# bark-simulator/planner-miqp

Hardware: AMD Instinct MI355X
Metric: MIQP solves/sec to 1% gap, 2-agent x 20-step x 32-region (higher is better)
Workload: dtype f64

## Files before the change

### planner_miqp_amd/csrc/as_onchip.hip

```cpp
namespace miqp {

#ifdef MIQP_PROFILE
#define ASP_T(var) const long long var = clock64()
#define ASP_ACC(k, t0, t1) asp_[k] += (unsigned long long)((t1) - (t0))
#else
#define ASP_T(var)
#define ASP_ACC(k, t0, t1)
#endif
constexpr int AS_MAXSTEP = 220;
constexpr double AS_VTOL = 1.0e-8;
constexpr double AS_DEP = 1.0e-8;
constexpr int AS_MT = 64;
constexpr int AS_MSTR = AS_MT * (AS_MT + 1) / 2;

__host__ __device__ constexpr bool as_shape_ok(int C, int N) { return (C == 1 || C == 2) && N >= 1 && N <= 2 * OC_NSL; }

template <int C> __device__ inline int as_col(int pq) { return C == 2 ? ((pq & 3) << 2) | (pq >> 2) : ((pq & 1) << 2) | (pq >> 1); }
template <int C> __device__ inline int as_pcol(int q) { return C == 2 ? ((q & 3) << 2) | (q >> 2) : ((q & 3) << 1) | (q >> 2); }

template <int C, int NSL, int GCAP = miqp::OC_GCAP>
__global__ void __launch_bounds__(64, (GCAP > 128 ? 1 : 2)) as_onchip_kernel(DevBuf B) {
  static_assert(C == 1 || C == 2, "a stage of 16 columns holds the chains of up to two cars");
  constexpr bool CM = true;
  constexpr bool BIG = GCAP > 128;
  constexpr int OC_GCAP = GCAP, OC_GSLOTS = OC_GCAP / 64, OC_GCOEF = oc_gcoef_of(OC_GCAP);
  constexpr int NX = 6 * C, NZ = 8 * C, NCH = 2 * C;
  const Layout& Y = B.Y;
  const int tid = threadIdx.x, lg = tid >> 4, lc = tid & 15;
  const int par = lg >> 1, side = lg & 1;
  const double bsgn = side ? -1.0 : 1.0;
  WAVE_DUMP(BIG ? 1 : 4);
  const int* const clist = BIG && B.cls_take ? B.cls_list + (size_t)(B.cls_take - 1) * B.batch_cap : nullptr;
  const int nbatch = clist ? (B.cls_count[B.cls_take - 1] < B.batch_cap ? B.cls_count[B.cls_take - 1] : B.batch_cap) : (*B.batch_count < B.batch_cap ? *B.batch_count : B.batch_cap);
  const int N = Y.N, NSLOT = Y.NSLOT;
  extern __shared__ double lds[];
  char* const L0 = (char*)lds;
  const OcLds LL = oc_lds_layout(N, Y.fixlen, OC_GCAP, !BIG);
  double* const Z = (double*)(L0 + LL.z);
  double* const scr = (double*)(L0 + LL.u);
  double* const V = (double*)(L0 + LL.u);
  unsigned long long* const bkey = (unsigned long long*)(L0 + LL.r);
  const int SPAN = LL.gmeta - LL.u;
  double* const kref = (double*)(L0 + LL.u + SPAN - N * 32);
  double* const kff = kref - N * 4;
  double* const KS = kff - N * 16;
  const int STG_CAP = (SPAN - N * 192) / 8;
  uint4* const gmeta = (uint4*)(L0 + LL.gmeta);
  double* const gcoef = (double*)(L0 + LL.gcoef);
  double* const grhs = (double*)(L0 + LL.grhs);
  double* const Wd = (double*)(L0 + LL.wd);
  int* const sstart = (int*)(L0 + LL.sstart);
  unsigned short* const cand = (unsigned short*)(L0 + LL.cand);
  signed char* const fix = (signed char*)(L0 + LL.fix);
  __shared__ int sh_node;
  __shared__ unsigned long long sh_stat[32];
  if (tid < 32) sh_stat[tid] = 0ull;
  const unsigned long long lt = (1ull << tid) - 1ull;

  const int chunk = B.as_chunk > 0 ? B.as_chunk : 1;
  int run_next = 0, run_end = 0;
  const int quota = BIG ? 0 : B.as_quota; int handed = 0;
#ifdef MIQP_PROFILE
  const unsigned long long wv_c0 = __builtin_amdgcn_s_memtime(), wv_r0 = __builtin_amdgcn_s_memrealtime();
  unsigned long long wv_first = 0; int wv_nodes = 0;
  if (!BIG && tid == 0) wv_first = atomicMin(&B.prof[120], wv_r0);
#endif
  for (;;) {
    __syncthreads();
    if (run_next >= run_end) {
      if (quota > 0 && handed >= quota) break;
      ++handed;
      if (tid == 0) sh_node = atomicAdd(B.work_counter, chunk);
      __syncthreads();
      run_next = __builtin_amdgcn_readfirstlane(sh_node); run_end = run_next + chunk;
      if (run_next >= nbatch) break;
    }
    const int slot_ = run_next++;
    if (slot_ >= nbatch) { run_next = run_end; continue; }
    const int node = clist ? __builtin_amdgcn_readfirstlane(clist[slot_]) : slot_;
    {
      const int cls = B.batch_large ? (int)B.batch_large[node] : (is_probe_word(B.batch_depth[node]) ? 1 : 0);
      if (cls != (BIG ? 1 : 0)) continue;
    }
    WAVE_DUMP_NODE();
    const int inst = __builtin_amdgcn_readfirstlane(B.batch_inst[node]);
    const double* D = B.inst_d + (size_t)inst * Y.dstride;
    const int* T = B.inst_i + (size_t)inst * Y.istride;
    const double ts = D[Y.d_glob + 7];
    const double aqs = 2.0 * D[Y.d_misc + 0];
    const double iaq = aqs > 0.0 ? 1.0 / aqs : 0.0;
    {
      const signed char* src = B.pool_fix + (size_t)B.batch_node[node] * Y.fixlen;
      for (int k = tid; k < Y.fixlen; k += 64) fix[k] = src[k];
      if (tid < 16) Wd[tid] = tid < NZ ? D[Y.d_wd + oc_lcol<C, CM>(as_pcol<C>(tid))] : 0.0;
      for (int k = tid; k < N * 32; k += 64) bkey[k] = ~0ull;
      for (int k = tid; k <= N + 1; k += 64) sstart[k] = 0;
    }
    __syncthreads();
    const double* Rf = D + Y.d_ref;
    double cutoff = 1e300;
    {
      const double inc0 = fmin(inc_from_key(*(volatile unsigned long long*)&B.inc_key[inst]), B.inc_ext[inst]);
      const double gap_ = is_probe_word(B.batch_depth[node]) ? 0.0 : B.inst_gap[inst];
      if (B.use_cutoff && inc0 < 1e300) cutoff = inc0 - gap_ * (1e-10 + fabs(inc0)) - B.inst_const[inst];
    }

#ifdef MIQP_PROFILE
    unsigned long long asp_[12] = {0, 0, 0, 0, 0, 0, 0, 0, 0, 0, 0, 0};
#endif
    ASP_T(ta0);
    int ngen = 0;
    {
      unsigned long long* const bmp = (unsigned long long*)scr;
      const int nw = (N * NSLOT + 63) >> 6;
      unsigned short* const pre = (unsigned short*)(bmp + nw);
      for (int k = tid; k < nw; k += 64) bmp[k] = 0ull;
      OC_WAVE_SYNC();
      const int cls_off[8] = {0, 7, 11, 16, 16 + Y.EL, 16 + 5 * Y.EL, C * Y.SC, C * Y.SC + 8 * Y.NP};
      const int cls_cnt[8] = {7, 4, 5, Y.EL, 4 * Y.EL, 5 * Y.O, 8 * Y.NP, 16 * Y.NP};
      auto take = [&](int i, int slot) {
        if (decode_row<C, false>(Y, D, T, fix, i, slot, nullptr).active) {
          int col; double sg, rh;
          if (box_of_slot<C>(Y, D, T, fix, i, slot, col, sg, rh)) atomicMin(&bkey[(i * 2 + (sg < 0.0 ? 1 : 0)) * 16 + as_col<C>(oc_pcol<C, CM>(col))], d2key(rh));
          else { const int pcode = i * NSLOT + slot; atomicOr(&bmp[pcode >> 6], 1ull << (pcode & 63)); }
        }
      };
      unsigned short* const plist = pre + ((nw + 1 + 3) & ~3);
      const int LCAP = (int)(((char*)(L0 + LL.r) - (char*)plist) / 2) - 64;
      int nlist = 0;
      auto flush = [&]() {
        OC_WAVE_SYNC();
        for (int j0 = 0; j0 < nlist; j0 += 64) if (j0 + tid < nlist) { const int pc = plist[j0 + tid]; const int i = pc / NSLOT; take(i, pc - i * NSLOT); }
        OC_WAVE_SYNC();
        nlist = 0;
      };
      for (int e0 = 0; e0 < C * N; e0 += 64) {
        const int e = e0 + tid;
        if (e < C * N) {
          const int c = e / N, i = e - c * N;
          const double* G = D + Y.d_glob;
          const int code = i >= 1 ? (int)fix[Y.f_reg + c * N + i] : -1;
          const unsigned int skip = i >= 1 ? (unsigned int)T[Y.i_boxskip + c * N + i] : 0x7Fu;
          const double* rt = code >= 0 ? D + Y.d_reg + (c * Y.P + (code >> 2)) * REGSZ : nullptr;
          const double* Hc = (!rt && i >= 1) ? region_hull(Y, D, T, fix, c, i) : nullptr;
          auto put = [&](int col, bool neg, double rh) { atomicMin(&bkey[(i * 2 + (neg ? 1 : 0)) * 16 + as_col<C>(oc_pcol<C, CM>(col))], d2key(rh)); };
          if (i >= 1) {
            const double a_lo_x = rt ? rt[11] : Hc[0], a_hi_x = rt ? rt[12] : Hc[1], a_lo_y = rt ? rt[13] : Hc[2], a_hi_y = rt ? rt[14] : Hc[3];
            if (!(skip & 1u)) put(6 * c + 1, true, -G[0]);
            if (!(skip & 2u)) put(6 * c + 4, true, -G[0]);
            if (!(skip & 4u)) put(6 * c + 1, false, G[1]);
            if (!(skip & 8u)) put(6 * c + 2, false, a_hi_x);
            if (!(skip & 16u)) put(6 * c + 2, true, -a_lo_x);
            if (!(skip & 32u)) put(6 * c + 5, false, a_hi_y);
            if (!(skip & 64u)) put(6 * c + 5, true, -a_lo_y);
          }
          if (i <= N - 2) {
#pragma unroll
            for (int s_ = 0; s_ < 2; ++s_) {
              double lo, hi;
              if (i == 0) { lo = D[Y.d_u0box + c * 4 + 2 * s_]; hi = D[Y.d_u0box + c * 4 + 2 * s_ + 1]; }
              else if (rt) { lo = rt[15 + 2 * s_]; hi = rt[16 + 2 * s_]; }
              else { lo = Hc[4 + 2 * s_]; hi = Hc[5 + 2 * s_]; }
              put(6 * C + 2 * c + s_, false, hi); put(6 * C + 2 * c + s_, true, -lo);
            }
          }
        }
      }
#pragma unroll 1
      for (int cl = 0; cl < 8; ++cl) {
#ifdef MIQP_PROFILE
        if (cl == 2) { const long long tq_ = clock64(); asp_[9] += (unsigned long long)(tq_ - ta0); }
#endif
        const int cnt = cls_cnt[cl], off = cls_off[cl];
        const bool percar = cl < 6;
        const int per = percar ? C * cnt : cnt, total = N * per;
        for (int e0 = 0; e0 < total; e0 += 64) {
          const int e = e0 + tid;
          int i = 0, slot = 0; bool in = e < total;
          if (in) { i = e / per; const int rem = e - i * per; slot = percar ? (rem / cnt) * Y.SC + off + rem % cnt : off + rem; }
          if (cl < 2) continue;
          const bool cnd = in && slot_maybe<C>(Y, fix, i, slot);
          const unsigned long long mk = __ballot(cnd);
          if (cnd) plist[nlist + __popcll(mk & lt)] = (unsigned short)(i * NSLOT + slot);
          nlist += __popcll(mk);
          if (nlist > LCAP) flush();
        }
      }
      flush();
      if (tid == 0) { int a = 0; for (int k = 0; k < nw; ++k) { pre[k] = (unsigned short)(a < 65535 ? a : 65535); a += __popcll(bmp[k]); } pre[nw] = (unsigned short)(a < 65535 ? a : 65535); }
      OC_WAVE_SYNC();
      ngen = pre[nw];
      if (ngen <= OC_GCAP)
        for (int k = tid; k < nw; k += 64) {
          unsigned long long bits = bmp[k]; int pos = pre[k];
          while (bits) { const int b = __ffsll((long long)bits) - 1; cand[pos++] = (unsigned short)(k * 64 + b); bits &= bits - 1ull; }
        }
      OC_WAVE_SYNC();
    }
#ifdef MIQP_PROFILE
    const long long tq1_ = clock64();
#endif
    bool overflow = ngen > OC_GCAP;
    int ncoef = 0;
    for (int c0 = 0; c0 < ngen && !overflow; c0 += OC_SCR) {
      double* g = scr + (tid & (OC_SCR - 1)) * OC_SSTR;
      RowOut r; r.active = false; r.rhs = 0; r.aq = 0;
      int i = 0, nn = 0;
      const bool mine = tid < OC_SCR && c0 + tid < ngen;
      int slot_ = 0;
      if (mine) { const int pcode = cand[c0 + tid]; i = pcode / NSLOT; slot_ = pcode - i * NSLOT; r = decode_row<C, true>(Y, D, T, fix, i, slot_, g); }
      unsigned long long map = 0ull; unsigned int cols = 0u;
      double v6[6];
#pragma unroll
      for (int k = 0; k < 6; ++k) v6[k] = 0.0;
      if (mine) {
        for (int q = 0; q < NZ; ++q) {
          const double v = g[q];
          if (v != 0.0 && nn < 6) {
#pragma unroll
            for (int k = 0; k < 6; ++k) if (k == nn) v6[k] = v;
            const int pq = as_col<C>(oc_pcol<C, CM>(q));
            map |= (unsigned long long)(nn + 1) << (4 * pq); cols |= (unsigned int)pq << (4 * nn); nn++;
          }
        }
      }
      const bool keep = mine && nn > 0;
      const unsigned long long mk = __ballot(keep);
      const unsigned long long b0 = __ballot(keep && (nn & 1)), b1 = __ballot(keep && (nn & 2)), b2 = __ballot(keep && (nn & 4));
      const int tot = __popcll(b0) + 2 * __popcll(b1) + 4 * __popcll(b2);
      if (ncoef + tot > OC_GCOEF) { overflow = true; break; }
      if (keep) {
        const int idx = sstart[N + 1] + __popcll(mk & lt);
        const int off = ncoef + __popcll(b0 & lt) + 2 * __popcll(b1 & lt) + 4 * __popcll(b2 & lt);
#pragma unroll
        for (int k = 0; k < 6; ++k) if (k < nn) gcoef[off + k] = v6[k];
        uint4 m4; m4.x = (unsigned int)map; m4.y = (unsigned int)(map >> 32);
        m4.z = (unsigned int)off | ((unsigned int)nn << 16) | ((unsigned int)i << 20) | (r.aq > 0.0 ? 0x80000000u : 0u); m4.w = cols;
        gmeta[idx] = m4; grhs[idx] = r.rhs;
        cand[idx] = (unsigned short)(i * NSLOT + slot_);
      }
      OC_WAVE_SYNC();
      if (tid == 0) sstart[N + 1] += __popcll(mk);
      ncoef += tot;
      OC_WAVE_SYNC();
    }
    if (overflow) {
      if (B.batch_A) B.batch_A[(size_t)node * 64 + tid] = 0xFFFFu;
      if (tid == 0) {
        if (B.ring_M) B.batch_Mtag[node] = 0ull;
        B.batch_ok[node] = 5; B.pool_big[B.batch_node[node]] |= (BIG ? 2 : 1); if (B.stats) { atomicAdd(&B.stats[3], 1ull); atomicAdd(&B.stats[8 + (ngen >= 512 ? 15 : ngen / 32)], 1ull); }
      }
      continue;
    }
    const int NM = sstart[N + 1];
    OC_WAVE_SYNC();

    ASP_T(ta1); ASP_ACC(0, ta0, ta1);
#ifdef MIQP_PROFILE
    asp_[11] += (unsigned long long)(ta1 - tq1_);
#endif
    double brhs[NSL];
    unsigned int bact = 0u, binA = 0u, ginA = 0u;
#pragma unroll
    for (int k = 0; k < NSL; ++k) {
      const int i = 2 * k + par;
      brhs[k] = 1e300;
      if (i < N && lc < NZ) {
        const unsigned long long key = bkey[(i * 2 + side) * 16 + lc];
        if (key != ~0ull) { brhs[k] = key2d(key); bact |= 1u << k; }
      }
    }
    OC_WAVE_SYNC();

    const double h1 = ts, h2 = 0.5 * ts * ts, h3 = ts * ts * ts / 6.0;
    const double* const tb = D + Y.d_astab;
    if constexpr (C == 2) {
      for (int k = tid; k < N * 16; k += 64) KS[k] = tb[k];
      for (int k = tid; k < N * 4; k += 64) kref[k] = tb[N * 16 + k];
    } else {
      for (int k = tid; k < N * 8; k += 64) KS[(k >> 3) * 16 + (k & 7)] = tb[k];
      for (int k = tid; k < N * 2; k += 64) kref[(k >> 1) * 4 + (k & 1)] = tb[N * 8 + k];
    }
    OC_WAVE_SYNC();
    typedef double d2_t __attribute__((ext_vector_type(2)));
    auto subst = [&](const bool fromx0, const int itop, const int iend, double* const out) {
      for (int k = tid; k < (N - 1) * 4; k += 64) if ((k >> 2) > itop) kff[k] = fromx0 ? kref[k] : 0.0;
      if (tid < NCH) {
        const int ch = tid;
        double p0 = 0.0, p1 = 0.0, p2 = 0.0;
        int i0 = itop;
        if (itop >= N - 1) { const d2_t a = *(const d2_t*)(V + (N - 1) * 16 + 4 * ch); p0 = a[0]; p1 = a[1]; p2 = V[(N - 1) * 16 + 4 * ch + 2]; i0 = N - 2; }
        if (i0 >= 0) {
          d2_t va = *(const d2_t*)(V + i0 * 16 + 4 * ch), vb = *(const d2_t*)(V + i0 * 16 + 4 * ch + 2);
          d2_t ka = *(const d2_t*)(KS + (i0 * 4 + ch) * 4), kb = *(const d2_t*)(KS + (i0 * 4 + ch) * 4 + 2);
          double kr = fromx0 ? kref[i0 * 4 + ch] : 0.0;
          for (int i = i0; i >= 0; --i) {
            const int j = i > 0 ? i - 1 : 0;
            const d2_t nva = *(const d2_t*)(V + j * 16 + 4 * ch), nvb = *(const d2_t*)(V + j * 16 + 4 * ch + 2);
            const d2_t nka = *(const d2_t*)(KS + (j * 4 + ch) * 4), nkb = *(const d2_t*)(KS + (j * 4 + ch) * 4 + 2);
            const double nkr = fromx0 ? kref[j * 4 + ch] : 0.0;
            const double su = vb[1] + h3 * p0 + h2 * p1 + h1 * p2;
            const double sx0 = va[0] + p0, sx1 = va[1] + h1 * p0 + p1, sx2 = vb[0] + h2 * p0 + h1 * p1 + p2;
            kff[i * 4 + ch] = fma(su, kb[1], kr);
            p0 = sx0 - ka[0] * su; p1 = sx1 - ka[1] * su; p2 = sx2 - kb[0] * su;
            va = nva; vb = nvb; ka = nka; kb = nkb; kr = nkr;
          }
        }
      }
      OC_WAVE_SYNC();
      if (tid < NCH) {
        const int ch = tid;
        double x0 = 0.0, x1 = 0.0, x2 = 0.0;
        if (fromx0) { const int c = ch >> 1, s = ch & 1; x0 = D[Y.d_x0 + 6 * c + 3 * s]; x1 = D[Y.d_x0 + 6 * c + 3 * s + 1]; x2 = D[Y.d_x0 + 6 * c + 3 * s + 2]; }
        const int ie = iend < N - 1 ? iend : N - 2;
        d2_t ka = *(const d2_t*)(KS + ch * 4), kb = *(const d2_t*)(KS + ch * 4 + 2);
        double kf = kff[ch];
        for (int i = 0; i <= ie; ++i) {
          const int j = i < N - 2 ? i + 1 : N - 2;
          const d2_t nka = *(const d2_t*)(KS + (j * 4 + ch) * 4), nkb = *(const d2_t*)(KS + (j * 4 + ch) * 4 + 2);
          const double nkf = kff[j * 4 + ch];
          const double u = -kf - (ka[0] * x0 + ka[1] * x1 + kb[0] * x2);
          d2_t oa, ob; oa[0] = x0; oa[1] = x1; ob[0] = x2; ob[1] = u;
          *(d2_t*)(out + i * 16 + 4 * ch) = oa; *(d2_t*)(out + i * 16 + 4 * ch + 2) = ob;
          const double n0 = x0 + h1 * x1 + h2 * x2 + h3 * u, n1 = x1 + h1 * x2 + h2 * u, n2 = x2 + h1 * u;
          x0 = n0; x1 = n1; x2 = n2;
          ka = nka; kb = nkb; kf = nkf;
        }
        if (iend >= N - 1 || ie == N - 2) { d2_t oa, ob; oa[0] = x0; oa[1] = x1; ob[0] = x2; ob[1] = 0.0; *(d2_t*)(out + (ie + 1) * 16 + 4 * ch) = oa; *(d2_t*)(out + (ie + 1) * 16 + 4 * ch + 2) = ob; }
// ... 434 lines not shown
```

### planner_miqp_amd/csrc/solve_diag.hpp

```cpp
#pragma once

inline void debug_sync(hipStream_t st, int round, const char* stage, int nodes = -1) {
  hipError_t e_ = hipStreamSynchronize(st);
  if (nodes >= 0) std::fprintf(stderr, "[dbg] round %d %s (%d nodes): %s\n", round, stage, nodes, hipGetErrorString(e_));
  else std::fprintf(stderr, "[dbg] round %d %s: %s\n", round, stage, hipGetErrorString(e_));
}

inline bool trace_selection(const DevCtx& X, int rounds, int bc) {
  const DevBuf& B = X.B;
  std::vector<double> sb(bc); std::vector<int> sd(bc); double io_ = 0; int md_ = 0;
  HIP_OK(hipMemcpy(sb.data(), B.batch_bound, (size_t)bc * 8, hipMemcpyDeviceToHost)); HIP_OK(hipMemcpy(sd.data(), B.batch_depth, (size_t)bc * 4, hipMemcpyDeviceToHost));
  HIP_OK(hipMemcpy(&io_, B.inc_obj, 8, hipMemcpyDeviceToHost)); HIP_OK(hipMemcpy(&md_, B.inst_mode, 4, hipMemcpyDeviceToHost));
  std::vector<int> ord(bc); for (int k = 0; k < bc; ++k) ord[k] = k;
  std::sort(ord.begin(), ord.end(), [&](int a, int b) { return sd[a] != sd[b] ? sd[a] > sd[b] : sb[a] < sb[b]; });
  std::fprintf(stderr, "[sel] r%d mode %d incumbent %a:", rounds, md_, io_);
  for (int k : ord) std::fprintf(stderr, " %d.%d/%a", sd[k] >> 6, sd[k] & 63, sb[k]);
  std::fprintf(stderr, "\n");
  return true;
}

inline bool trace_batch(const DevCtx& X, int rounds, int bc) {
  const DevBuf& B = X.B; hipStream_t st = X.stream;
  HIP_OK(hipStreamSynchronize(st));
  if (X.stream2) HIP_OK(hipStreamSynchronize(X.stream2));
// ... 36 lines not shown
  hipEvent_t e0, e1; HIP_OK(hipEventCreate(&e0)); HIP_OK(hipEventCreate(&e1));
  HIP_OK(hipEventRecord(e0, st));
  for (int r = 0; r < replay; ++r) launch_ipm_batch(X, B, bc, st);
  HIP_OK(hipEventRecord(e1, st)); HIP_OK(hipStreamSynchronize(st));
  float ms = 0; HIP_OK(hipEventElapsedTime(&ms, e0, e1));
  std::vector<int> its(bc); HIP_OK(hipMemcpy(its.data(), B.batch_it, (size_t)bc * 4, hipMemcpyDeviceToHost));
  long long tot = 0; for (int v : its) tot += v;
  std::fprintf(stderr, "[miqp_gpu replay] %d nodes, %lld node-iterations: %.3f ms per pass, %.1f ns per node-iteration\n", bc, tot, ms / replay, 1e6 * ms / replay / (double)tot);
#ifdef MIQP_ABLATE
  if (X.oc_grid > 0 && Y.C == 2) {
    const size_t l_oc = (size_t)oc_lds_layout(Y.N, Y.fixlen).total;
    auto run = [&](auto kern, int mask) {
      HIP_OK(hipFuncSetAttribute((const void*)kern, hipFuncAttributeMaxDynamicSharedMemorySize, (int)l_oc));
      auto once = [&] { (void)hipMemsetAsync(B.work_counter, 0, 4, st); (void)hipMemsetAsync(B.ovf_count, 0, 4, st); hipLaunchKernelGGL(kern, dim3(std::min(bc, X.oc_grid)), dim3(64), l_oc, st, B); };
      once(); HIP_OK(hipEventRecord(e0, st)); for (int r = 0; r < 3; ++r) once(); HIP_OK(hipEventRecord(e1, st)); HIP_OK(hipStreamSynchronize(st));
      float m2 = 0; HIP_OK(hipEventElapsedTime(&m2, e0, e1));
      std::fprintf(stderr, "[miqp_gpu ablate] mask %4d: %.3f ms per pass of %d nodes x 15 iterations = %.1f ns per node-iteration\n", mask, m2 / 3, bc, 1e6 * m2 / 3 / (bc * 15.0));
      return true;
    };
    run(ipm_onchip_kernel<2, OC_NSL, 1>, 1); run(ipm_onchip_kernel<2, OC_NSL, 3>, 3); run(ipm_onchip_kernel<2, OC_NSL, 5>, 5); run(ipm_onchip_kernel<2, OC_NSL, 9>, 9);
    run(ipm_onchip_kernel<2, OC_NSL, 17>, 17); run(ipm_onchip_kernel<2, OC_NSL, 33>, 33); run(ipm_onchip_kernel<2, OC_NSL, 65>, 65); run(ipm_onchip_kernel<2, OC_NSL, 129>, 129);
    run(ipm_onchip_kernel<2, OC_NSL, 257>, 257); run(ipm_onchip_kernel<2, OC_NSL, 513>, 513); run(ipm_onchip_kernel<2, OC_NSL, 1023>, 1023);
    run(ipm_onchip_kernel<2, OC_NSL, 1025>, 1025);
    launch_ipm_batch(X, B, bc, st);
  }
#endif
  replay = 0;
  return true;
}

inline bool print_progress(const DevCtx& X, double t, int rounds, long long launched_nodes, double const0) {
  const DevBuf& B = X.B; hipStream_t st = X.stream;
  double lb0 = 0, io0 = 0; int oc0 = 0; unsigned long long k0 = 0;
  HIP_OK(hipMemcpyAsync(&lb0, B.lower_bound, 8, hipMemcpyDeviceToHost, st)); HIP_OK(hipMemcpyAsync(&io0, B.inc_obj, 8, hipMemcpyDeviceToHost, st));
  HIP_OK(hipMemcpyAsync(&oc0, B.open_count, 4, hipMemcpyDeviceToHost, st)); HIP_OK(hipMemcpyAsync(&k0, B.inc_key, 8, hipMemcpyDeviceToHost, st));
  int fc0 = 0; HIP_OK(hipMemcpyAsync(&fc0, B.far_count, 4, hipMemcpyDeviceToHost, st));
  HIP_OK(hipStreamSynchronize(st));
  std::fprintf(stderr, "[miqp_gpu] t %.2f s round %d nodes %lld: instance 0 bound %.4f incumbent %.4f open %d + %d\n", t, rounds, launched_nodes, lb0, k0 >= 0xFFF0000000000000ull ? INFINITY : io0 + const0, oc0, fc0);
  return true;
}

inline bool dump_open_list(const DevCtx& X, const char* dp, int rounds, int NS, double const0) {
  const DevBuf& B = X.B; const Layout& Y = X.Y; const int open_cap = X.open_cap;
  int oc0 = 0; HIP_OK(hipMemcpy(&oc0, B.open_count, 4, hipMemcpyDeviceToHost)); oc0 = std::min(oc0, open_cap);
  const size_t src = ((size_t)(rounds & 1) * NS + 0) * open_cap;
  std::vector<double> hb(oc0); std::vector<int> hn(oc0), hd(oc0);
  if (oc0 > 0) { HIP_OK(hipMemcpy(hb.data(), B.open_bound + src, (size_t)oc0 * 8, hipMemcpyDeviceToHost)); HIP_OK(hipMemcpy(hn.data(), B.open_node + src, (size_t)oc0 * 4, hipMemcpyDeviceToHost));
    HIP_OK(hipMemcpy(hd.data(), B.open_depth + src, (size_t)oc0 * 4, hipMemcpyDeviceToHost)); }
  std::vector<int> ord(oc0); for (int k = 0; k < oc0; ++k) ord[k] = k;
  std::sort(ord.begin(), ord.end(), [&](int x, int y) { return hb[x] < hb[y]; });
  if (FILE* f = std::fopen(dp, "w")) {
    std::fprintf(f, "%d %d %d %d %d %d %d\n", oc0, Y.fixlen, Y.f_reg, Y.f_env, Y.f_obs, Y.f_c2c, Y.N);
    std::vector<signed char> rec(Y.fixlen);
    for (int q = 0; q < std::min(oc0, 400); ++q) {
      int k = ord[q]; HIP_OK(hipMemcpy(rec.data(), B.pool_fix + (size_t)hn[k] * Y.fixlen, Y.fixlen, hipMemcpyDeviceToHost));
      std::fprintf(f, "%.9g %d", hb[k] + const0, hd[k] >> 6); for (int x = 0; x < Y.fixlen; ++x) std::fprintf(f, " %d", (int)rec[x]); std::fprintf(f, "\n");
    }
    std::fclose(f);
  }
  return true;
}

#ifdef MIQP_PROFILE
inline bool print_profile(const DevCtx& X) {
  const DevBuf& B = X.B;
  { unsigned long long pf[64]; HIP_OK(hipMemcpy(pf, B.prof + 64, 64 * 8, hipMemcpyDeviceToHost));
    const char* nm[10] = {"decode", "rowpass", "bw.phi", "bw.TS+p", "bw.readlane+LDL", "bw.Ksolve", "bw.update", "forward", "step", "update"};
    double tot = 0; for (int q = 0; q < 10; ++q) tot += (double)pf[q];
    { unsigned long long po[16]; HIP_OK(hipMemcpy(po, B.prof, 16 * 8, hipMemcpyDeviceToHost));
      const char* no[9] = {"build", "bw.rows/assemble", "bw.mfma", "bw.TS", "bw.cholK", "bw.P", "forward", "step", "update"};
      double to = 0; for (int q = 0; q < 9; ++q) to += (double)po[q];
      if (po[10]) { std::fprintf(stderr, "[miqp_gpu profile] memory-backed kernel nodes %llu iters %llu cycles/node-iter %.0f :", po[10], po[9], to / std::max(1ull, po[9]));
        for (int q = 0; q < 9; ++q) std::fprintf(stderr, " %s %.1f%% (%.0f)", no[q], 100.0 * po[q] / to, (double)po[q] / std::max(1ull, po[9]));
        std::fprintf(stderr, "; inside bw.TS, the stage-Hessian chain: weights + staging %.0f, single-entry rows %.0f, MFMA loop %.0f, reductions + diagonal %.0f", (double)po[12] / std::max(1ull, po[9]), (double)po[13] / std::max(1ull, po[9]), (double)po[14] / std::max(1ull, po[9]), (double)po[15] / std::max(1ull, po[9]));
        std::fprintf(stderr, "\n"); } }
    std::fprintf(stderr, "[miqp_gpu profile] on-chip nodes %llu iters %llu cycles/node-iter %.0f :", pf[11], pf[10], tot / std::max(1ull, pf[10]));
    for (int q = 0; q < 10; ++q) std::fprintf(stderr, " %s %.1f%% (%.0f)", nm[q], 100.0 * pf[q] / tot, (double)pf[q] / std::max(1ull, pf[10]));
    std::fprintf(stderr, "\n");
    { unsigned long long pa[14]; HIP_OK(hipMemcpy(pa, B.prof + 80, 14 * 8, hipMemcpyDeviceToHost));
      const char* na[9] = {"decode", "gains + first iterate", "scan", "response of the row", "q", "directions + ratio test + M update", "iterate refresh", "results", "warm start"};
      double ta = 0; for (int q = 0; q < 9; ++q) ta += (double)pa[q];
      if (pa[10]) { std::fprintf(stderr, "[miqp_gpu profile] active-set kernel nodes %llu steps %llu cycles/node %.0f :", pa[10], pa[11], ta / (double)pa[10]);
        for (int q = 0; q < 9; ++q) std::fprintf(stderr, " %s %.1f%% (%.0f)", na[q], 100.0 * pa[q] / ta, (double)pa[q] / (double)pa[10]);
        std::fprintf(stderr, "; inside the decode: bound classes %.0f, general-row pass %.0f", (double)pa[12] / (double)pa[10], (double)pa[13] / (double)pa[10]);
        std::fprintf(stderr, "\n");
        unsigned long long pw[3], pl[6]; HIP_OK(hipMemcpy(pw, B.prof + 94, 3 * 8, hipMemcpyDeviceToHost)); HIP_OK(hipMemcpy(pl, B.prof + 120, 6 * 8, hipMemcpyDeviceToHost));
        if (pw[2] && pw[1] && pl[5]) std::fprintf(stderr, "[miqp_gpu profile] standard active-set launches: %llu wavefronts resident %.0f shader cycles = %.1f us each (shader clock %.0f MHz); per launch (%llu folded): span %.3f ms, from the first wavefront out of work to the last end %.3f ms, wavefronts %.0f, resident wavefront time / (span x wavefronts) %.3f\n",
          pw[2], (double)pw[0] / pw[2], (double)pw[1] / pw[2] / 100.0, 100.0 * (double)pw[0] / (double)pw[1], pl[5], (double)pl[3] / pl[5] / 1e5, (double)pl[4] / pl[5] / 1e5, (double)pw[2] / pl[5], ((double)pw[1]) / ((double)pl[3] * ((double)pw[2] / pl[5])));
        unsigned long long ph[16]; HIP_OK(hipMemcpy(ph, B.prof + 128, 16 * 8, hipMemcpyDeviceToHost));
        if (pw[2]) { std::fprintf(stderr, "[miqp_gpu profile] standard active-set wavefronts by their start after the launch's first (< 0.05 / 0.2 / 0.5 / 1 / 2 / 4 / 8 ms / later), %% :");
          for (int q = 0; q < 8; ++q) std::fprintf(stderr, " %.1f", 100.0 * ph[q] / pw[2]);
          std::fprintf(stderr, "; by the nodes they solved (0 / <= 4 / <= 16 / <= 32 / <= 64 / more), %% :");
          for (int q = 8; q < 14; ++q) std::fprintf(stderr, " %.1f", 100.0 * ph[q] / pw[2]);
          std::fprintf(stderr, "\n"); }
        if (const char* wd = X.sw.wave_dump) {
          std::vector<unsigned long long> w(4 * 4 * 4096); HIP_OK(hipMemcpy(w.data(), B.prof + 160, w.size() * 8, hipMemcpyDeviceToHost));
          if (FILE* f = std::fopen(wd, "w")) { for (int q = 0; q < 4 * 4096; ++q) if (w[4 * q]) std::fprintf(f, "%d %llu %llu %u %u %llu %d\n", q & 4095, w[4 * q], w[4 * q + 1], (unsigned)(w[4 * q + 2] >> 32), (unsigned)w[4 * q + 2], w[4 * q + 3], q >> 12); std::fclose(f); } } } }
    { unsigned long long pe[8]; HIP_OK(hipMemcpy(pe, B.prof + 100, 8 * 8, hipMemcpyDeviceToHost));
      const char* ne[6] = {"load", "regions", "leaf disjunctions", "branching", "lifting + reservation", "records"};
      double te = 0; for (int q = 0; q < 6; ++q) te += (double)pe[q];
      if (pe[6]) { std::fprintf(stderr, "[miqp_gpu profile] eval_kernel, %llu branched nodes, cycles/node %.0f :", pe[6], te / (double)pe[6]);
        for (int q = 0; q < 6; ++q) std::fprintf(stderr, " %s %.1f%% (%.0f)", ne[q], 100.0 * pe[q] / te, (double)pe[q] / (double)pe[6]);
        std::fprintf(stderr, "\n"); } }
    { unsigned long long ps[10]; HIP_OK(hipMemcpy(ps, B.prof + 110, 10 * 8, hipMemcpyDeviceToHost));
      const char* ns[8] = {"incumbent copy / kill", "setup", "pass 1 (prune, keys)", "far refill", "bound reduce + spill select", "focus + window + share", "radix select + ties", "pass 3 (emit, compact)"};
      double ts = 0; for (int q = 0; q < 8; ++q) ts += (double)ps[q];
      if (ps[8]) { std::fprintf(stderr, "[miqp_gpu profile] select_kernel, %llu workgroups that reached the end (thread 0's clock), mean list %.0f entries, cycles each %.0f :", ps[8], (double)ps[9] / (double)ps[8], ts / (double)ps[8]);
        for (int q = 0; q < 8; ++q) std::fprintf(stderr, " %s %.1f%% (%.0f)", ns[q], 100.0 * ps[q] / ts, (double)ps[q] / (double)ps[8]);
        std::fprintf(stderr, "\n"); } }
    HIP_OK(hipMemset(B.prof, 0, 160 * 8)); }
  return true;
}
#endif

inline bool print_stats(const DevCtx& X) {
  const DevBuf& B = X.B; const Layout& Y = X.Y;
  unsigned long long hs[256]; HIP_OK(hipMemcpy(hs, B.stats, sizeof(hs), hipMemcpyDeviceToHost)); HIP_OK(hipMemset(B.stats, 0, sizeof(hs)));
  const double nn_ = (double)std::max(1ull, hs[0]);
  std::fprintf(stderr, "[miqp_gpu stats] on-chip nodes %llu (general rows %.1f, coefficients %.1f, box keys %.1f, iterations %.1f per node), handed over %llu; general rows / 32 histogram:", hs[0], hs[1] / nn_, hs[4] / nn_, hs[2] / nn_, hs[5] / nn_, hs[3]);
  for (int q = 0; q < 16; ++q) std::fprintf(stderr, " %llu", hs[8 + q]);
  std::fprintf(stderr, "\n");
  std::fprintf(stderr, "[miqp_gpu stats] node outcomes: infeasible %llu (%.1f it), cut off %llu (%.1f it), not converged %llu (%.1f it), solved %llu (%.1f it) of which: bound >= incumbent %llu, within gap %llu, integer feasible %llu, branched %llu (%.2f children; by kind region/env/obstacle/car-car: %llu x %.1f, %llu x %.1f, %llu x %.1f, %llu x %.1f)\n",
               hs[32], hs[36] / (double)std::max(1ull, hs[32]), hs[33], hs[37] / (double)std::max(1ull, hs[33]), hs[34], hs[38] / (double)std::max(1ull, hs[34]), hs[35], hs[39] / (double)std::max(1ull, hs[35]),
               hs[40], hs[41], hs[42], hs[43], hs[44] / (double)std::max(1ull, hs[43]), hs[48], hs[52] / (double)std::max(1ull, hs[48]), hs[49], hs[53] / (double)std::max(1ull, hs[49]),
               hs[50], hs[54] / (double)std::max(1ull, hs[50]), hs[51], hs[55] / (double)std::max(1ull, hs[51]));
  std::fprintf(stderr, "[miqp_gpu stats] region sets: tightened at %llu (car, step) sites, %llu nodes closed because a step had no region left; children not created because of their lifted bound %llu (multi-row lift larger than the single-row one: %llu), car/car sets tightened at %llu groups\n", hs[58], hs[59], hs[56], hs[57], hs[61]);
  std::fprintf(stderr, "[miqp_gpu stats] region branchings flagged by: own rows %llu (worst class acc box %llu, jerk box %llu, sector %llu, half-plane %llu, curvature %llu, slow square %llu), environment front rows %llu, obstacle front rows %llu, car/car front rows %llu; by step:",
               hs[64], hs[70], hs[71], hs[72], hs[73], hs[74], hs[75], hs[65], hs[66], hs[67]);
  for (int q = 0; q < 32 && q < Y.N; ++q) std::fprintf(stderr, " %llu", hs[160 + q]);
  std::fprintf(stderr, "\n[miqp_gpu stats] node outcomes by origin (processed: infeasible / cut off / not converged / solved):");
  const char* on_[16] = {"root|reg-ref", "reg-adjacent", "reg-other", "reg-slow", "env-ref", "env-other", "-", "-", "obs-ref", "obs-other", "-", "-", "c2c-ref", "c2c-other", "-", "probe"};
  for (int q = 0; q < 16; ++q) if (hs[80 + q]) std::fprintf(stderr, " %s %llu: %llu / %llu / %llu / %llu;", on_[q], hs[80 + q], hs[96 + q], hs[112 + q], hs[128 + q], hs[144 + q]);
  std::fprintf(stderr, "\n[miqp_gpu stats] infeasible rounding probes re-rounded: %llu", hs[62]);
  std::fprintf(stderr, "\n[miqp_gpu stats] handed-over nodes with >= 480 general rows: %llu, mean %.0f, most %llu general rows", hs[7], (double)hs[6] / std::max(1ull, hs[7]), hs[5]);
  std::fprintf(stderr, "\n[miqp_gpu stats] rounding probes by iterations / 3 (0-2, 3-5, ..., 45+):");
  { const char* oc_n[4] = {"infeasible", "cut off", "not converged", "solved"};
    for (int o = 0; o < 4; ++o) { std::fprintf(stderr, " %s", oc_n[o]); for (int q = 0; q < 16; ++q) std::fprintf(stderr, " %llu", hs[192 + 16 * o + q]); std::fprintf(stderr, ";"); } }
  std::fprintf(stderr, "\n");
  return true;
}

inline void print_as_stats(const unsigned long long* h_as) {
  std::fprintf(stderr, "[miqp_gpu stats] active-set launch: %llu nodes (%.1f steps, %.1f drops, %.1f rows from the parent's active set, %.1f active rows at the end per node; %llu infeasible, %llu cut off; %llu started from the parent's M, %llu fell back to a cold start), %llu handed to the interior point (no free slot %llu, step cap %llu, curvature %llu, down-date pivot %llu, rows off their equalities %llu, other %llu); M rebuilt because: the parent left none %llu, the ring had come round %llu, another row count %llu; in the larger block %llu nodes (%.1f steps), of them leaves of the local search %llu (%.1f steps), rounding probes %llu; by their general rows (<= 64 / 96 / 128 / 192 / more) %llu / %llu / %llu / %llu / %llu\n",
               h_as[0], h_as[1] / (double)std::max(1ull, h_as[0]), h_as[3] / (double)std::max(1ull, h_as[0]), h_as[7] / (double)std::max(1ull, h_as[0]), h_as[6] / (double)std::max(1ull, h_as[0]), h_as[4], h_as[5], h_as[8], h_as[9], h_as[2], h_as[11], h_as[12], h_as[13], h_as[14], h_as[15], h_as[10], h_as[17], h_as[18], h_as[19], h_as[20], h_as[21] / (double)std::max(1ull, h_as[20]), h_as[22], h_as[23] / (double)std::max(1ull, h_as[22]), h_as[29], h_as[24], h_as[25], h_as[26], h_as[27], h_as[28]);
}
```

Before: 1085.

## Decode constraint rows per lane-site with count-scan-write instead of slot enumeration

Replaces the slot-by-slot decode of the active-set kernel with a per-site decode: each lane owns one (step, car) or (step, pair) site, emits box bounds to atomic keys and counts general rows, then a wave prefix scan assigns output offsets and a second pass writes the packed rows. This removes the bitmap, candidate list, per-slot ballots and the scratch-based coefficient extraction loop. It decodes each site twice and leaves lanes idle when there are fewer sites than lanes. Under a debug macro the old path stays available and both images are hashed and compared.

Result: no change. 1098, median of 3 (+1.2%).

```diff
diff --git a/planner_miqp_amd/csrc/as_onchip.hip b/planner_miqp_amd/csrc/as_onchip.hip
--- a/planner_miqp_amd/csrc/as_onchip.hip
+++ b/planner_miqp_amd/csrc/as_onchip.hip
@@ -1,3 +1,5 @@
+#include "site_decode.hpp"
+
 namespace miqp {
 
 #ifdef MIQP_PROFILE
@@ -110,6 +112,120 @@
 #endif
     ASP_T(ta0);
     int ngen = 0;
+    bool overflow = false;
+    struct SdCount {
+      unsigned long long* bkey; int ncand, nkeep, ncoef;
+      __device__ void box(int i, int col, double sgn, double rhs) { atomicMin(&bkey[(i * 2 + (sgn < 0.0 ? 1 : 0)) * 16 + as_col<C>(oc_pcol<C, true>(col))], d2key(rhs)); }
+      __device__ void gen(int, int, double, double, int, double a0, double a1, double a2, double a3, double a4, double a5, int bb, double b0, double b1, double b2, double b3, double b4, double b5) {
+        int nn = (a0 != 0.0) + (a1 != 0.0) + (a2 != 0.0) + (a3 != 0.0) + (a4 != 0.0) + (a5 != 0.0);
+        if (bb >= 0) nn += (b0 != 0.0) + (b1 != 0.0) + (b2 != 0.0) + (b3 != 0.0) + (b4 != 0.0) + (b5 != 0.0);
+        if (nn > 6) nn = 6;
+        ++ncand;
+        if (nn > 0) { ++nkeep; ncoef += nn; }
+      }
+    };
+    struct SdWrite {
+      uint4* gmeta; double* gcoef; double* grhs; unsigned short* cand; int NSLOT, idx, off;
+      __device__ void box(int, int, double, double) {}
+      __device__ void gen(int i, int slot, double rhs, double aq, int ba, double a0, double a1, double a2, double a3, double a4, double a5, int bb, double b0, double b1, double b2, double b3, double b4, double b5) {
+        int nn = 0; unsigned long long map = 0ull; unsigned int cols = 0u;
+        auto put = [&](const int q, const double v) {
+          if (v != 0.0 && nn < 6) {
+            if (off + nn < OC_GCOEF) gcoef[off + nn] = v;
+            const int pq = as_col<C>(oc_pcol<C, true>(q));
+            map |= (unsigned long long)(nn + 1) << (4 * pq); cols |= (unsigned int)pq << (4 * nn); nn++;
+          }
+        };
+        put(ba, a0); put(ba + 1, a1); put(ba + 2, a2); put(ba + 3, a3); put(ba + 4, a4); put(ba + 5, a5);
+        if (bb >= 0) { put(bb, b0); put(bb + 1, b1); put(bb + 2, b2); put(bb + 3, b3); put(bb + 4, b4); put(bb + 5, b5); }
+        if (nn > 0 && idx < OC_GCAP) {
+          uint4 m4; m4.x = (unsigned int)map; m4.y = (unsigned int)(map >> 32);
+          m4.z = (unsigned int)off | ((unsigned int)nn << 16) | ((unsigned int)i << 20) | (aq > 0.0 ? 0x80000000u : 0u); m4.w = cols;
+          gmeta[idx] = m4; grhs[idx] = rhs; cand[idx] = (unsigned short)(i * NSLOT + slot);
+          ++idx; off += nn;
+        }
+      }
+    };
+#ifdef MIQP_PROFILE
+    long long tq1_ = 0;
+#endif
+    auto decode_sites = [&]() {
+      constexpr int SPS = C == 2 ? 3 : 1;
+      const int ln = fresh_lane();
+      const int si = ln / SPS, sj = ln - si * SPS;
+      const bool car_site = si < N && sj < C, pair_site = C == 2 && si < N && sj == C;
+      SdCount S1; S1.bkey = bkey; S1.ncand = 0; S1.nkeep = 0; S1.ncoef = 0;
+      if (car_site) {
+        const int c = sj, i = si;
+        const double* G = D + Y.d_glob;
+        const int code = i >= 1 ? (int)fix[Y.f_reg + c * N + i] : -1;
+        const unsigned int skip = i >= 1 ? (unsigned int)T[Y.i_boxskip + c * N + i] : 0x7Fu;
+        const double* rt = code >= 0 ? D + Y.d_reg + (c * Y.P + (code >> 2)) * REGSZ : nullptr;
+        const double* Hc = (!rt && i >= 1) ? region_hull(Y, D, T, fix, c, i) : nullptr;
+        auto put = [&](int col, bool neg, double rh) { atomicMin(&bkey[(i * 2 + (neg ? 1 : 0)) * 16 + as_col<C>(oc_pcol<C, CM>(col))], d2key(rh)); };
+        if (i >= 1) {
+          const double a_lo_x = rt ? rt[11] : Hc[0], a_hi_x = rt ? rt[12] : Hc[1], a_lo_y = rt ? rt[13] : Hc[2], a_hi_y = rt ? rt[14] : Hc[3];
+          if (!(skip & 1u)) put(6 * c + 1, true, -G[0]);
+          if (!(skip & 2u)) put(6 * c + 4, true, -G[0]);
+          if (!(skip & 4u)) put(6 * c + 1, false, G[1]);
+          if (!(skip & 8u)) put(6 * c + 2, false, a_hi_x);
+          if (!(skip & 16u)) put(6 * c + 2, true, -a_lo_x);
+          if (!(skip & 32u)) put(6 * c + 5, false, a_hi_y);
+          if (!(skip & 64u)) put(6 * c + 5, true, -a_lo_y);
+        }
+        if (i <= N - 2) {
+#pragma unroll
+          for (int s_ = 0; s_ < 2; ++s_) {
+            double lo, hi;
+            if (i == 0) { lo = D[Y.d_u0box + c * 4 + 2 * s_]; hi = D[Y.d_u0box + c * 4 + 2 * s_ + 1]; }
+            else if (rt) { lo = rt[15 + 2 * s_]; hi = rt[16 + 2 * s_]; }
+            else { lo = Hc[4 + 2 * s_]; hi = Hc[5 + 2 * s_]; }
+            put(6 * C + 2 * c + s_, false, hi); put(6 * C + 2 * c + s_, true, -lo);
+          }
+        }
+        site_rows_car<C>(Y, D, T, fix, c, i, S1);
+      } else if (pair_site) site_rows_pair<C>(Y, D, T, fix, 0, si, S1);
+      int pk = S1.nkeep, pc = S1.ncoef, pn = S1.ncand;
+#pragma unroll
+      for (int d = 1; d < 64; d <<= 1) {
+        const int tk = __shfl_up(pk, d), tc = __shfl_up(pc, d), tn = __shfl_up(pn, d);
+        if (tid >= d) { pk += tk; pc += tc; pn += tn; }
+      }
+      ngen = __shfl(pn, 63);
+      const int nkeep = __shfl(pk, 63), ncoef = __shfl(pc, 63);
+      overflow = ngen > OC_GCAP || ncoef > OC_GCOEF;
+#ifdef MIQP_PROFILE
+      { const long long tq_ = clock64(); asp_[9] += (unsigned long long)(tq_ - ta0); tq1_ = tq_; }
+#endif
+      if (overflow) return;
+      SdWrite S2; S2.gmeta = gmeta; S2.gcoef = gcoef; S2.grhs = grhs; S2.cand = cand; S2.NSLOT = NSLOT; S2.idx = pk - S1.nkeep; S2.off = pc - S1.ncoef;
+      if (car_site) site_rows_car<C>(Y, D, T, fix, sj, si, S2);
+      else if (pair_site) site_rows_pair<C>(Y, D, T, fix, 0, si, S2);
+      if (tid == 0) sstart[N + 1] = nkeep;
+      OC_WAVE_SYNC();
+    };
+#ifndef MIQP_DECODE_CHECK
+    decode_sites();
+#else
+    auto image_hash = [&]() -> unsigned long long {
+      unsigned long long hsh = 0x9E3779B97F4A7C15ull;
+      auto word = [&](const unsigned long long v) { hsh = (hsh ^ v) * 0x100000001B3ull; hsh ^= hsh >> 29; };
+      const int NMi = overflow ? 0 : sstart[N + 1];
+      for (int k = 0; k < N * 32; ++k) word(bkey[k]);
+      word((unsigned long long)(overflow ? 1 : 0)); word((unsigned long long)ngen);
+      if (!overflow) {
+        word((unsigned long long)NMi);
+        for (int k = 0; k < NMi; ++k) {
+          const uint4 m4 = gmeta[k]; word(((unsigned long long)m4.y << 32) | m4.x); word(((unsigned long long)m4.w << 32) | m4.z);
+          word((unsigned long long)__double_as_longlong(grhs[k])); word((unsigned long long)cand[k]);
+          const int off = (int)(m4.z & 0xFFFFu), nn = (int)((m4.z >> 16) & 7u);
+          for (int j = 0; j < nn; ++j) word((unsigned long long)__double_as_longlong(gcoef[off + j]));
+        }
+      }
+      return hsh;
+    };
+    auto decode_slots = [&]() {
+    ngen = 0;
     {
       unsigned long long* const bmp = (unsigned long long*)scr;
       const int nw = (N * NSLOT + 63) >> 6;
@@ -168,9 +284,6 @@
       }
 #pragma unroll 1
       for (int cl = 0; cl < 8; ++cl) {
-#ifdef MIQP_PROFILE
-        if (cl == 2) { const long long tq_ = clock64(); asp_[9] += (unsigned long long)(tq_ - ta0); }
-#endif
         const int cnt = cls_cnt[cl], off = cls_off[cl];
         const bool percar = cl < 6;
         const int per = percar ? C * cnt : cnt, total = N * per;
@@ -197,10 +310,7 @@
         }
       OC_WAVE_SYNC();
     }
-#ifdef MIQP_PROFILE
-    const long long tq1_ = clock64();
-#endif
-    bool overflow = ngen > OC_GCAP;
+    overflow = ngen > OC_GCAP;
     int ncoef = 0;
     for (int c0 = 0; c0 < ngen && !overflow; c0 += OC_SCR) {
       double* g = scr + (tid & (OC_SCR - 1)) * OC_SSTR;
@@ -244,6 +354,25 @@
       ncoef += tot;
       OC_WAVE_SYNC();
     }
+      if (!overflow) OC_WAVE_SYNC();
+    };
+    {
+      decode_sites();
+      OC_WAVE_SYNC();
+      unsigned long long h_sites = 0ull;
+      if (tid == 0) h_sites = image_hash();
+      OC_WAVE_SYNC();
+      for (int k = tid; k < N * 32; k += 64) bkey[k] = ~0ull;
+      for (int k = tid; k <= N + 1; k += 64) sstart[k] = 0;
+      for (int k = tid; k < OC_GCAP; k += 64) { gmeta[k] = make_uint4(0u, 0u, 0u, 0u); grhs[k] = 0.0; cand[k] = 0; }
+      for (int k = tid; k < OC_GCOEF; k += 64) gcoef[k] = 0.0;
+      OC_WAVE_SYNC();
+      decode_slots();
+      OC_WAVE_SYNC();
+      if (tid == 0) { sh_stat[30] += 1ull; sh_stat[31] += image_hash() != h_sites ? 1ull : 0ull; }
+      OC_WAVE_SYNC();
+    }
+#endif
     if (overflow) {
       if (B.batch_A) B.batch_A[(size_t)node * 64 + tid] = 0xFFFFu;
       if (tid == 0) {
diff --git a/planner_miqp_amd/csrc/site_decode.hpp b/planner_miqp_amd/csrc/site_decode.hpp
--- /dev/null
+++ b/planner_miqp_amd/csrc/site_decode.hpp
@@ -0,0 +1,159 @@
+namespace miqp {
+
+__device__ inline void sd_point(double& rhs, double& x0, double& x1, double& x3, double& x4, const double* rt, int t, double al, double be, const double* K) {
+  x0 += al;
+  if (t != PT_R) {
+    if (rt) { const double* p = rt + 19 + (t == PT_U ? 0 : 3); rhs -= al * p[0]; x1 += al * p[1]; x4 += al * p[2]; }
+    else if (al != 0.0) rhs -= al * K[(t == PT_U ? 0 : 2) + (al > 0.0 ? 0 : 1)];
+  }
+  x3 += be;
+  if (t != PT_R) {
+    if (rt) { const double* p = rt + 25 + (t == PT_U ? 0 : 3); rhs -= be * p[0]; x1 += be * p[1]; x4 += be * p[2]; }
+    else if (be != 0.0) rhs -= be * K[(t == PT_U ? 4 : 6) + (be > 0.0 ? 0 : 1)];
+  }
+}
+
+template <class Sink>
+__device__ inline void sd_edge(Sink& S, int i, int slot, int c, const double* rt, int pt, int tx, int ty, const double* ed) {
+  const double al = ed[0], be = ed[1], ga = ed[2];
+  if (pt == 0) {
+    if (be == 0.0 && fabs(al) == 1.0) { S.box(i, 6 * c, al, ga); return; }
+    if (al == 0.0 && fabs(be) == 1.0) { S.box(i, 6 * c + 3, be, ga); return; }
+    double x0 = 0.0, x3 = 0.0;
+    x0 += al; x3 += be;
+    S.gen(i, slot, ga, 0.0, 6 * c, x0, 0.0, 0.0, x3, 0.0, 0.0, -1, 0.0, 0.0, 0.0, 0.0, 0.0, 0.0);
+    return;
+  }
+  double rhs = ga, x0 = 0.0, x1 = 0.0, x3 = 0.0, x4 = 0.0;
+  x0 += al;
+  { const double* p = rt + 19 + (tx == PT_U ? 0 : 3); rhs -= al * p[0]; x1 += al * p[1]; x4 += al * p[2]; }
+  x3 += be;
+  { const double* p = rt + 25 + (ty == PT_U ? 0 : 3); rhs -= be * p[0]; x1 += be * p[1]; x4 += be * p[2]; }
+  S.gen(i, slot, rhs, 0.0, 6 * c, x0, x1, 0.0, x3, x4, 0.0, -1, 0.0, 0.0, 0.0, 0.0, 0.0, 0.0);
+}
+
+template <int C, class Sink>
+__device__ inline void site_rows_car(const Layout& Y, const double* D, const int* T, const signed char* fix, int c, int i, Sink& S) {
+  if (i < 1) return;
+  const int N = Y.N, sb = c * Y.SC;
+  const double* G = D + Y.d_glob;
+  const int code = (int)fix[Y.f_reg + c * N + i];
+  const double* rt = code >= 0 ? D + Y.d_reg + (c * Y.P + (code >> 2)) * REGSZ : nullptr;
+  if (code < 0) {
+    const double* Hc = D + Y.d_hull + (c * N + i) * HULLSZ;
+    if (Hc[14] != 0.0) {
+#pragma unroll
+      for (int k = 0; k < 2; ++k) S.gen(i, sb + 11 + k, Hc[10 + 3 * k], 0.0, 6 * c, 0.0, Hc[8 + 3 * k], 0.0, 0.0, Hc[9 + 3 * k], 0.0, -1, 0.0, 0.0, 0.0, 0.0, 0.0, 0.0);
+    }
+  } else {
+    const int h = code & 3;
+    if (h == 3) {
+#pragma unroll
+      for (int k = 0; k < 4; ++k) S.box(i, 6 * c + (k < 2 ? 1 : 4), (k & 1) ? -1.0 : 1.0, G[6]);
+    } else {
+      S.gen(i, sb + 11, 0.0, 0.0, 6 * c, 0.0, rt[0], 0.0, 0.0, rt[1], 0.0, -1, 0.0, 0.0, 0.0, 0.0, 0.0, 0.0);
+      S.gen(i, sb + 12, 0.0, 0.0, 6 * c, 0.0, rt[2], 0.0, 0.0, rt[3], 0.0, -1, 0.0, 0.0, 0.0, 0.0, 0.0, 0.0);
+      { const int* hs = T + Y.i_hs + ((c * Y.P + (code >> 2)) * 2 + h) * 2; S.box(i, 6 * c + (hs[0] == 0 ? 1 : 4), -(double)hs[1], -G[6]); }
+      S.gen(i, sb + 14, rt[5], 0.0, 6 * c, 0.0, -rt[6], -rt[4], 0.0, -rt[7], 1.0, -1, 0.0, 0.0, 0.0, 0.0, 0.0, 0.0);
+      S.gen(i, sb + 15, -rt[8], 0.0, 6 * c, 0.0, rt[9], rt[4], 0.0, rt[10], -1.0, -1, 0.0, 0.0, 0.0, 0.0, 0.0, 0.0);
+    }
+  }
+  const int dom = code >= 0 ? T[Y.i_dom + (c * Y.P + (code >> 2)) * 4 + (code & 3)] : 0;
+  if (Y.E >= 1) {
+    const signed char* fe = fix + Y.f_env + (c * N + i) * 5;
+    const int e0 = Y.E == 1 ? 0 : (int)fe[0], e1 = Y.E == 1 ? 0 : (int)fe[1], e2 = Y.E == 1 ? 0 : (int)fe[2], e3 = Y.E == 1 ? 0 : (int)fe[3], e4 = Y.E == 1 ? 0 : (int)fe[4];
+#pragma unroll
+    for (int pt = 0; pt < 5; ++pt) {
+      const int e = pt == 0 ? e0 : pt == 1 ? e1 : pt == 2 ? e2 : pt == 3 ? e3 : e4;
+      if (e < 0 || (pt > 0 && code < 0)) continue;
+      const int tx = pt == 0 ? PT_R : ((pt == 1 || pt == 3) ? PT_U : PT_L), ty = pt == 0 ? PT_R : (pt <= 2 ? PT_U : PT_L);
+      const int ne = T[Y.i_envn + e] < Y.EL ? T[Y.i_envn + e] : Y.EL;
+      for (int k = 0; k < ne; ++k) {
+        const double* ed = D + Y.d_env + (e * Y.EL + k) * 3;
+        if (pt > 0) {
+          int txs, tys;
+          if (corner_dominated(tx, ty, ed[0], ed[1], dom, txs, tys)) {
+            const int ps = env_corner(txs, tys);
+            if ((ps == 1 ? e1 : ps == 2 ? e2 : ps == 3 ? e3 : e4) == e) continue;
+          }
+        }
+        sd_edge(S, i, sb + 16 + pt * Y.EL + k, c, rt, pt, tx, ty, ed);
+      }
+    }
+  }
+  for (int o = 0; o < Y.O; ++o) {
+    const signed char* fo = fix + Y.f_obs + ((c * Y.O + o) * N + i) * 5;
+    const int k0 = (int)fo[0], k1 = (int)fo[1], k2 = (int)fo[2], k3 = (int)fo[3], k4 = (int)fo[4];
+#pragma unroll
+    for (int pt = 0; pt < 5; ++pt) {
+      const int kk = pt == 0 ? k0 : pt == 1 ? k1 : pt == 2 ? k2 : pt == 3 ? k3 : k4;
+      if (kk < 0 || kk >= Y.L || (pt > 0 && code < 0)) continue;
+      const int tx = pt == 0 ? PT_R : ((pt == 2 || pt == 4) ? PT_U : PT_L), ty = pt == 0 ? PT_R : (pt >= 3 ? PT_U : PT_L);
+      const double* ed = D + Y.d_obs + ((o * N + i) * Y.L + kk) * 3;
+      if (pt > 0) {
+        int txs, tys;
+        if (corner_dominated(tx, ty, ed[0], ed[1], dom, txs, tys)) {
+          const int ps = obs_corner(txs, tys);
+          if ((ps == 1 ? k1 : ps == 2 ? k2 : ps == 3 ? k3 : k4) == kk) continue;
+        }
+      }
+      sd_edge(S, i, sb + 16 + 5 * Y.EL + o * 5 + pt, c, rt, pt, tx, ty, ed);
+    }
+  }
+}
+
+template <int C, class Sink>
+__device__ inline void site_rows_pair(const Layout& Y, const double* D, const int* T, const signed char* fix, int p, int i, Sink& S) {
+  if (C < 2 || i < 1) return;
+  const int N = Y.N;
+  int c1, c2; pair_cars(p, C, c1, c2);
+  const int code1 = (int)fix[Y.f_reg + c1 * N + i], code2 = (int)fix[Y.f_reg + c2 * N + i];
+  const double* rt1 = code1 >= 0 ? D + Y.d_reg + (c1 * Y.P + (code1 >> 2)) * REGSZ : nullptr;
+  const double* rt2 = code2 >= 0 ? D + Y.d_reg + (c2 * Y.P + (code2 >> 2)) * REGSZ : nullptr;
+  const signed char* fc = fix + Y.f_c2c + (p * N + i) * 4;
+  const signed char* fn = fix + Y.f_c2n + (p * N + i) * 4;
+  const double Dsep = D[Y.d_dsep + p * N + i], Ssl = D[Y.d_ssl + i], smax = D[Y.d_smax + i], wsl = D[Y.d_misc + 0];
+  const double* K1 = (code1 < 0 && !Y.relax_front_off) ? region_fpk(Y, D, T, fix, c1, i) : nullptr;
+  const double* K2 = (code2 < 0 && !Y.relax_front_off) ? region_fpk(Y, D, T, fix, c2, i) : nullptr;
+  auto row = [&](const int slot, const int grp, const int alt, const int which, const bool excl) {
+    const bool need1 = grp >= 2, need2 = (grp == 1 || grp == 3);
+    if (need1 && code1 < 0 && (excl || !K1)) return;
+    if (need2 && code2 < 0 && (excl || !K2)) return;
+    const bool soft = (grp == 0 || grp == 3);
+    if (!excl) {
+      if (!soft && which == 1) return;
+      if (soft && which == 1 && !(smax > 0 && wsl > 0)) return;
+    }
+    const bool isx = alt < 2, lo = (alt == 0 || alt == 2);
+    const bool af = (grp < 2) == lo;
+    const int ta = grp == 0 ? PT_R : (grp == 3 ? PT_U : (lo ? PT_R : PT_U)), tb = grp == 0 ? PT_R : (grp == 3 ? PT_L : (lo ? PT_L : PT_R));
+    const double al = isx ? 1.0 : 0.0, be = isx ? 0.0 : 1.0;
+    double rhs = soft ? (which == 0 ? -(Dsep + Ssl) + smax : -(Dsep + Ssl)) : -Dsep;
+    const double aq = (!excl && soft && which == 1) ? 2.0 * wsl : 0.0;
+    double a0 = 0.0, a1 = 0.0, a3 = 0.0, a4 = 0.0, b0 = 0.0, b1 = 0.0, b3 = 0.0, b4 = 0.0;
+    sd_point(rhs, a0, a1, a3, a4, af ? rt1 : rt2, ta, al, be, af ? K1 : K2);
+    sd_point(rhs, b0, b1, b3, b4, af ? rt2 : rt1, tb, -al, -be, af ? K2 : K1);
+    double u0 = af ? a0 : b0, u1 = af ? a1 : b1, u3 = af ? a3 : b3, u4 = af ? a4 : b4;
+    double v0 = af ? b0 : a0, v1 = af ? b1 : a1, v3 = af ? b3 : a3, v4 = af ? b4 : a4;
+    if (excl) { u0 = -u0; u1 = -u1; u3 = -u3; u4 = -u4; v0 = -v0; v1 = -v1; v3 = -v3; v4 = -v4; rhs = -rhs; }
+    S.gen(i, slot, rhs, aq, 6 * c1, u0, u1, 0.0, u3, u4, 0.0, 6 * c2, v0, v1, 0.0, v3, v4, 0.0);
+  };
+  const int s0 = C * Y.SC + p * 8;
+#pragma unroll 1
+  for (int grp = 0; grp < 4; ++grp) {
+    const int alt = (int)fc[grp];
+    if (alt < 0) continue;
+#pragma unroll 1
+    for (int which = 0; which < 2; ++which) row(s0 + 2 * grp + which, grp, alt, which, false);
+  }
+  const int s1 = C * Y.SC + Y.NP * 8 + p * 16;
+#pragma unroll 1
+  for (int grp = 0; grp < 4; ++grp) {
+    const int m = (int)fn[grp];
+    if (m <= 0) continue;
+#pragma unroll 1
+    for (int alt = 0; alt < 4; ++alt) if ((m >> alt) & 1) row(s1 + 4 * grp + alt, grp, alt, 1, true);
+  }
+}
+
+}
diff --git a/planner_miqp_amd/csrc/solve_diag.hpp b/planner_miqp_amd/csrc/solve_diag.hpp
--- a/planner_miqp_amd/csrc/solve_diag.hpp
+++ b/planner_miqp_amd/csrc/solve_diag.hpp
@@ -142,7 +142,7 @@
       double ta = 0; for (int q = 0; q < 9; ++q) ta += (double)pa[q];
       if (pa[10]) { std::fprintf(stderr, "[miqp_gpu profile] active-set kernel nodes %llu steps %llu cycles/node %.0f :", pa[10], pa[11], ta / (double)pa[10]);
         for (int q = 0; q < 9; ++q) std::fprintf(stderr, " %s %.1f%% (%.0f)", na[q], 100.0 * pa[q] / ta, (double)pa[q] / (double)pa[10]);
-        std::fprintf(stderr, "; inside the decode: bound classes %.0f, general-row pass %.0f", (double)pa[12] / (double)pa[10], (double)pa[13] / (double)pa[10]);
+        std::fprintf(stderr, "; inside the decode: site pass (bounds to their keys, general rows counted, scan over the lanes) %.0f, packing pass %.0f", (double)pa[12] / (double)pa[10], (double)pa[13] / (double)pa[10]);
         std::fprintf(stderr, "\n");
         unsigned long long pw[3], pl[6]; HIP_OK(hipMemcpy(pw, B.prof + 94, 3 * 8, hipMemcpyDeviceToHost)); HIP_OK(hipMemcpy(pl, B.prof + 120, 6 * 8, hipMemcpyDeviceToHost));
         if (pw[2] && pw[1] && pl[5]) std::fprintf(stderr, "[miqp_gpu profile] standard active-set launches: %llu wavefronts resident %.0f shader cycles = %.1f us each (shader clock %.0f MHz); per launch (%llu folded): span %.3f ms, from the first wavefront out of work to the last end %.3f ms, wavefronts %.0f, resident wavefront time / (span x wavefronts) %.3f\n",
@@ -203,4 +203,7 @@
 inline void print_as_stats(const unsigned long long* h_as) {
   std::fprintf(stderr, "[miqp_gpu stats] active-set launch: %llu nodes (%.1f steps, %.1f drops, %.1f rows from the parent's active set, %.1f active rows at the end per node; %llu infeasible, %llu cut off; %llu started from the parent's M, %llu fell back to a cold start), %llu handed to the interior point (no free slot %llu, step cap %llu, curvature %llu, down-date pivot %llu, rows off their equalities %llu, other %llu); M rebuilt because: the parent left none %llu, the ring had come round %llu, another row count %llu; in the larger block %llu nodes (%.1f steps), of them leaves of the local search %llu (%.1f steps), rounding probes %llu; by their general rows (<= 64 / 96 / 128 / 192 / more) %llu / %llu / %llu / %llu / %llu\n",
                h_as[0], h_as[1] / (double)std::max(1ull, h_as[0]), h_as[3] / (double)std::max(1ull, h_as[0]), h_as[7] / (double)std::max(1ull, h_as[0]), h_as[6] / (double)std::max(1ull, h_as[0]), h_as[4], h_as[5], h_as[8], h_as[9], h_as[2], h_as[11], h_as[12], h_as[13], h_as[14], h_as[15], h_as[10], h_as[17], h_as[18], h_as[19], h_as[20], h_as[21] / (double)std::max(1ull, h_as[20]), h_as[22], h_as[23] / (double)std::max(1ull, h_as[22]), h_as[29], h_as[24], h_as[25], h_as[26], h_as[27], h_as[28]);
-}
+#ifdef MIQP_DECODE_CHECK
+  std::fprintf(stderr, "[miqp_gpu decode check] nodes decoded both ways %llu, nodes whose LDS images differ %llu\n", h_as[30], h_as[31]);
+#endif
+}
```
